# ChristophReich1996/Multi-StyleGAN

Measured on AMD Instinct MI355X. Metric: training images/sec (G+D step, 256^2, seq=3x2ch), higher is better.
Workload: dtype bf16

## Files before the change

### include/msg_hip.h

```cpp
#ifndef MSG_HIP_H
#define MSG_HIP_H

#ifdef __cplusplus
extern "C" {
#endif

enum { MSG_OK = 0, MSG_EINVAL = -1, MSG_EUNSUPPORTED = -2, MSG_ELAUNCH = -3 };
enum { MSG_F32 = 0, MSG_BF16 = 1, MSG_F16 = 2, MSG_F64 = 3, MSG_F32_SPLIT = 4 };

#define MSG_ABI_VERSION 5
int msg_abi_version(void);
const char* msg_build_arch(void);
const char* msg_strerror(int code);

int msg_upfirdn2d(const void* x, const float* fir, void* y, int dtype,
                  int major, int in_h, int in_w, int minor, int kh, int kw,
                  int up_x, int up_y, int down_x, int down_y,
                  int pad_x0, int pad_x1, int pad_y0, int pad_y1, void* stream);

int msg_upfirdn2d_pitched(const void* x, const float* fir, void* y, int dtype,
                          int major, int in_h, int in_w, int minor, int in_pitch, int kh, int kw,
                          int up_x, int up_y, int down_x, int down_y,
                          int pad_x0, int pad_x1, int pad_y0, int pad_y1, void* stream);

// ... 54 lines not shown
                     int per_sample, int k_chunks, int oi_major, float gain,
                     float* ws, long long ws_floats, void* stream);
long long msg_conv2d_wgrad_workspace(int dtype, int B, int IH, int IW, int Cx, int I, int OH, int OW, int ldgy,
                                     int O, int ldgw, int kh, int kw, int stride, int pad, int pixel_shuffle,
                                     int per_sample, int k_chunks);

int msg_demod_coeff(const float* W, const float* s, float* d, int B, int O, int I, int taps,
                    float scale, float eps, void* stream);
int msg_scale_rows_cols(const float* base, const float* rowscale, const float* colscale, void* out,
                        int dtype, int B, int R, int T, int C, int Ck, float gain, void* stream);
int msg_modulate_weights(const float* base, const float* wsq, const float* style, void* out, float* d_out,
                         int dtype, int B, int R, int O, int T, int C, int Ck, float scale, float eps, void* stream);
int msg_modulate_backward(const float* gwk, const float* W, const float* s, const float* d, float* gW,
                          float* gs_part, int B, int O, int I, int taps, int ldg, int o_group,
                          float scale, void* stream);
int msg_scale_rows_cols2(const float* base, const float* row1, const float* col1, const float* row2, const float* col2,
                         void* out, int dtype, int B, int R, int T, int C, int Ck, float gain, void* stream);
int msg_modulate_backward2(const float* gwk, const float* W, const float* s, const float* d, const float* v,
                           float* gW, float* gs_part, int B, int O, int I, int taps, int ldg, int o_group,
                           float scale, void* stream);

int msg_relayout_weight(const float* w, void* fwd, void* dgrad, float* wsq, int dtype,
                        int O, int I, int T, int Ck, int Ok, int flip, int t_major, float gain, void* stream);

int msg_gather_taps(const void* x, void* y, int dtype, int B, int H, int W, int Cx, int C, int kh, int kw,
                    int pad, int Ko, void* stream);
int msg_fold_taps(const void* g, const void* add, void* gx, int dtype, int B, int H, int W, int Ko, int C, int kh, int kw,
                  int pad, int ldx, int ld_add, void* stream);

int msg_scaled_add(const void* a, const void* b, void* y, int dtype, long long n, float beta, float gain, void* stream);
int msg_rgb_skip_merge(const void* conv, int dtype, int ld, const float* bias, const float* skip, const float* fir,
                       float* out, int B, int C, int H, int W, void* stream);
int msg_rgb_skip_merge_backward(const float* g, void* g_conv, int dtype, int ld, float* g_skip, const float* fir,
                                int B, int C, int H, int W, void* stream);
int msg_gamma_merge(const void* a, const void* b, const float* gamma, void* y, int dtype, long long n, float gain, void* stream);
long long msg_gamma_merge_backward_workspace(void);
int msg_gamma_merge_backward(const void* gy, const void* a, const float* gamma, void* ga, void* gb, float* g_gamma, int dtype,
                             long long n, float gain, float* ws, void* stream);
int msg_scaled_add_rows(const void* a, const void* b, void* y, int dtype, long long rows, int cols,
                        long long lda, long long ldb, long long ldy, float beta, float gain, void* stream);

int msg_softmax_rows(const void* x, void* y, int dtype, long long rows, int cols, void* stream);
int msg_softmax_rows_backward(const void* y, const void* gy, void* gx, int dtype, long long rows, int cols,
                              void* stream);
int msg_softmax_rows_backward2(const void* y, const void* gy, const void* v, void* d_y, void* d_gy, int dtype,
                               long long rows, int cols, void* stream);

int msg_nonlocal_attention_supported(int B, int Nq, int Nk, int dk, int dv);
int msg_nonlocal_attention_fwd(const void* q, const void* k, const void* vt, void* o, float* lse, int dtype,
                               int B, int Nq, int Nk, int dk, int dv, void* stream);
int msg_maxpool2x2_fwd(const void* x, void* y, unsigned short* idx, int dtype, int B, int H, int W, int C, long long ldx,
                       void* stream);
int msg_maxpool2x2_bwd(const void* gy, const unsigned short* idx, void* gx, int dtype, int B, int H, int W, int C,
                       void* stream);
int msg_maxpool2x2_gather(const void* v, const unsigned short* idx, void* out, int dtype, int B, int H, int W, int C,
                          long long ldv, void* stream);

int msg_nonlocal_attention_bwd_splits(int B, int Nq, int Nk);
int msg_nonlocal_attention_bwd(const void* q, const void* qt, const void* k, const void* kt, const void* v,
                               const void* dO, const void* dOt, const void* o, const float* lse, float* delta,
                               void* dq, void* dk_out, void* dv_out, float* workspace, int dtype,
                               int B, int Nq, int Nk, int dk, int dv, void* stream);

int msg_affine_warp(const float* x, float* y, const float* angle_deg, float angle_const, const float* scale_xy,
                    const float* select_u, const float* p, int rot_prob, float cx, float cy, int padding,
                    int align_corners, int B, int C, int H, int W, int backward, void* workspace, void* stream);

long long msg_minibatch_stddev_workspace(int C, int H, int W, int groups, int dtype);
int msg_minibatch_stddev(const void* x, void* y, float* stat, float* workspace, int dtype,
                         int B, int C, int H, int W, int ldx, int ldy, int groups, float alpha, void* stream);
int msg_minibatch_stddev_backward(const void* x, const void* gy, const float* gstat, void* gx, int dtype,
                                  int B, int C, int H, int W, int ldx, int ldgy, int ldgx, int groups,
                                  float alpha, void* stream);

int msg_conv2d_fprop_act(const void* x, const void* w, void* y, int dtype,
                         int B, int IH, int IW, int Cx, int Ck, int OH, int OW, int N, int ldy,
                         int kh, int kw, int stride, int pad, long long w_batch_stride,
                         const float* act_bias, const float* noise, const float* noise_weight,
                         int noise_batch, float alpha, float scale, void* stream);
int msg_conv2d_fprop_act_mask(const void* x, const void* w, void* y, int dtype,
                              int B, int IH, int IW, int Cx, int Ck, int OH, int OW, int N, int ldy,
                              int kh, int kw, int stride, int pad, long long w_batch_stride,
                              const float* act_bias, const float* noise, const float* noise_weight,
                              int noise_batch, float alpha, float scale, unsigned char* mask, void* stream);

int msg_conv2d_fprop_residual(const void* x, const void* w, void* y, int dtype,
                              int B, int IH, int IW, int Cx, int Ck, int OH, int OW, int N, int ldy,
                              int kh, int kw, int stride, int pad, long long w_batch_stride,
                              const void* residual, int res_ld, float gain, void* stream);

int msg_conv2d_fprop_act_backward(const void* x, const void* w, void* y, int dtype,
                                  int B, int IH, int IW, int Cx, int Ck, int OH, int OW, int N, int ldy,
                                  int kh, int kw, int stride, int pad, long long w_batch_stride,
                                  const void* residual, int res_ld,
                                  const unsigned char* sign_mask, int mask_tile_m, int mask_tile_n,
                                  const void* sign_map, int sign_ld, float alpha, float scale,
                                  float* grad_bias, const float* noise, int noise_batch, float* grad_noise_weight,
                                  float* ws, long long ws_floats, void* stream);

int msg_act_pointwise_head(const void* x, const float* bias, const float* w, float* y, int dtype,
                           long long npix, int C, float wscale, float alpha, float scale, void* stream);
long long msg_act_pointwise_head_backward_workspace(long long npix, int C);
int msg_act_pointwise_head_backward(const void* x, const float* bias, const float* w, const float* gy, void* gx,
                                    float* grad_bias_and_w, int dtype, long long npix, int C, float wscale,
                                    float alpha, float scale, float* ws, long long ws_floats, void* stream);

int msg_linear_fprop(const float* x, const float* w, const float* bias, float* y, int M, int N, int K,
                     float gain, float bias_gain, void* stream);
int msg_linear_dgrad(const float* gy, const float* w, float* gx, int M, int N, int K, float gain, void* stream);
int msg_linear_wgrad(const float* gy, const float* x, float* gw, float* gb, int M, int N, int K,
                     float gain, float bias_gain, void* stream);

int msg_linear_grouped_fprop(const float* x, const int* slot, const float* const* w, const float* const* bias, float* y,
                             int G, int M, int N, int K, int L, float gain, float bias_gain, void* stream);
int msg_linear_grouped_dgrad(const float* gy, const float* const* w, float* gx, int G, int M, int N, int K, float gain,
                             void* stream);
int msg_linear_grouped_wgrad(const float* gy, const float* x, const int* slot, float* gw, float* gb, int G, int M, int N,
                             int K, int L, float gain, float bias_gain, void* stream);
int msg_linear_grouped_wgrad_ptrs(const float* gy, const float* x, const int* slot, float* const* gw, float* const* gb, int G,
                                  int M, int N, int K, int L, float gain, float bias_gain, void* stream);

enum {
    MSG_PLAN_REG = 0,
    MSG_PLAN_DMA = 1,
    MSG_PLAN_PP = 2,
    MSG_PLAN_ROW3 = 3,
    MSG_PLAN_ROW3N = 4,
    MSG_PLAN_THIN = 5,
    MSG_PLAN_UPCONV = 6,
    MSG_FPLAN_FIELDS = 5
};
int msg_conv2d_fprop_launch_plan(int dtype, int B, int IH, int IW, int Cx, int Ck, int OH, int OW, int N, int ldy,
                                 int kh, int kw, int stride, int pad, int in_up, int pixel_shuffle,
                                 long long w_batch_stride, int has_bias, int epilogue, long long* out, int n_out_fields);
enum {
    MSG_WPLAN_GENERIC = 0,
    MSG_WPLAN_DMA = 1,
    MSG_WPLAN_UNI = 2,
    MSG_WPLAN_ROW3 = 3,
    MSG_WPLAN_ROW3_W32 = 4,
    MSG_WPLAN_FIELDS = 11
};
int msg_conv2d_wgrad_plan(int dtype, int B, int IH, int IW, int Cx, int I, int OH, int OW, int ldgy,
                          int O, int ldgw, int kh, int kw, int stride, int pad, int pixel_shuffle,
                          int per_sample, int k_chunks, long long* out, int n_out_fields);
int msg_conv2d_fprop_plan(int dtype, int B, int IH, int IW, int Cx, int Ck, int OH, int OW, int N,
                          int kh, int kw, long long w_batch_stride);
long long msg_conv2d_fprop_act_backward_workspace(int dtype, int B, int IH, int IW, int Cx, int Ck, int OH, int OW,
                                                  int N, int kh, int kw, long long w_batch_stride, int has_noise);
int msg_conv2d_fprop_upconv_eligible(int B, int IH, int IW, int Cx, int Ck, int OH, int OW, int N, int kh, int kw,
                                     int stride, int pad, int in_up, int pixel_shuffle, long long w_batch_stride);
int msg_conv2d_fprop_thin_eligible(int B, int IH, int IW, int Cx, int Ck, int OH, int OW, int N, int ldy, int kh, int kw,
                                   int stride, int pad, int in_up, int pixel_shuffle, int act_mode);

int msg_flat_adam(float* param, const float* grad, float* exp_avg, float* exp_avg_sq, float* ema, long long n,
                  const float* coef, float lr, float beta1, float beta2, float eps, int step, float ema_decay,
                  void* stream);
int msg_flat_ema(float* ema, const float* param, long long n, float decay, void* stream);

long long msg_tlfm_prepare_workspace(int B, int T);
int msg_tlfm_prepare(const unsigned short* raw, const unsigned char* hflip, void* out, int dtype,
                     int B, int C, int T, int H, int W, int vflip,
                     float lo1, float div1, float lo2, float div2,
                     unsigned int* ws, void* stream);

int msg_tlfm_frame_range(const unsigned short* frames, long long N, int H, int W,
                         unsigned int* range, void* stream);
int msg_tlfm_gather(const unsigned short* frames, const unsigned int* range, long long N,
                    const int* index, const unsigned char* hflip, void* out, int dtype,
                    int B, int C, int T, int H, int W, int vflip,
                    float lo1, float div1, float lo2, float div2, void* stream);

long long msg_tlfm_export_workspace(int B, int T);
int msg_tlfm_export(const void* x, int dtype, const int* bf_range, unsigned short* out,
                    int B, int C, int T, int H, int W, int vflip, int bf_normalise,
                    float low1, float div1, float low2, float div2,
                    float* ws, void* stream);

int msg_sample_sheet(const void* seq, unsigned char* out, int dtype,
                     int B, int C, int T, int H, int W, int tints, void* stream);

enum { MSG_GAN_LOGISTIC = 0, MSG_GAN_WASSERSTEIN = 1, MSG_GAN_HINGE = 2 };
enum { MSG_GAN_AUX_NONE = 0, MSG_GAN_AUX_WEIGHT = 1, MSG_GAN_AUX_LABEL = 2 };
long long msg_gan_loss_workspace(long long n_real, long long n_fake);
int msg_gan_loss(const void* pred_real, const void* pred_fake, const float* aux, float* out, int dtype, int kind,
                 int aux_mode, long long n_real, long long n_fake, long long P, float* ws, long long ws_floats,
                 void* stream);
int msg_gan_loss_backward(const void* pred_real, const void* pred_fake, const float* aux, const float* grad_out,
                          void* grad_real, void* grad_fake, int dtype, int kind, int aux_mode,
                          long long n_real, long long n_fake, long long P, void* stream);

#define MSG_ELASTIC_MAX_SIGMA 32
long long msg_elastic_workspace(int B, int H, int W);
int msg_elastic_deform(const void* in, const float* noise, float* field, void* out, int dtype,
                       int B, int F, int H, int W, int sigma, float alpha, void* ws, void* stream);

#define MSG_JPEG_MAX_WIDTH 16384
long long msg_jpeg_workspace(int N, int H, int W);
int msg_jpeg_scan_capacity(int N, int H, int W, long long* bytes);
int msg_jpeg_encode(const unsigned char* rgb, const unsigned short* qtables, short* coef, unsigned char* scan,
                    long long* offsets, int N, int H, int W, void* ws, void* stream);

enum { MSG_METRIC_NORM_NONE = 0, MSG_METRIC_NORM_SOURCE = 1, MSG_METRIC_NORM_RESIZED = 2 };
#define MSG_METRIC_MAX_SCALE 8
long long msg_metric_input_workspace(int B, int T, int H, int W, int t, int out_h, int out_w, int norm);
int msg_metric_input(const void* images, int in_dtype, int B, int C, int T, int H, int W,
                     int channel, int t, void* out, int out_dtype, int planes,
                     int out_h, int out_w, int norm, void* ws, void* stream);

#ifdef __cplusplus
}
#endif
#endif
```

### multi_stylegan_amd/csrc/conv_dispatch.h

```cpp
#pragma once
#include "msg_common.h"

struct ConvProblem {
    int dtype;
    int split;
    int B, IH, IW, Cx, Ck, OH, OW, N, ldy;
    int kh, kw, stride, pad, in_up, pixel_shuffle;
    long long w_batch_stride;

    bool per_sample() const { return w_batch_stride != 0; }
    int samples() const { return per_sample() ? B : 1; }
    long long mtot() const { return per_sample() ? (long long)OH * OW : (long long)B * OH * OW; }
    int esz() const { return dtype == MSG_BF16 ? 2 : 4; }
    long long x_bstride() const { return (long long)IH * IW * Cx; }
    long long y_bstride() const { return (pixel_shuffle ? 4ll : 1ll) * OH * OW * ldy; }
    long long x_bytes() const { return (long long)(per_sample() ? 1 : B) * IH * IW * Cx * esz(); }
    long long w_bytes() const { return (long long)N * kh * kw * Ck * esz(); }
    bool fits31() const { return x_bytes() < 0x7ffffff0ll && w_bytes() < 0x7ffffff0ll; }
};

enum ConvKernel {
    CONV_THIN_N, CONV_THIN_K,
    CONV_UPCONV,
    CONV_ROW3, CONV_ROW3N,
    CONV_PP,
    CONV_DMA, CONV_REG, CONV_REG_LEAN, CONV_REG_SPLIT
};

struct ConvPlan {
    ConvKernel kernel;
    int tile_m, tile_n;
    bool supported;
};

inline int conv_act_mode(const ActEpilogue* act) { return act ? act->enabled : 0; }

template <typename P>
inline void conv_fill_common(P& p, const ConvProblem& q, const ActEpilogue* act) {
    p.B = q.B; p.IH = q.IH; p.IW = q.IW; p.Cx = q.Cx; p.Ck = q.Ck; p.OH = q.OH; p.OW = q.OW; p.N = q.N; p.ldy = q.ldy;
    p.per_sample = q.per_sample();
    if (act) p.act = *act;
    p.x_bstride = q.x_bstride();
    p.w_bstride = q.w_batch_stride;
    p.y_bstride = q.y_bstride();
    p.Mtot = (int)q.mtot();
}
template <typename P>
inline void conv_fill_taps(P& p, const ConvProblem& q) {
    p.kh = q.kh; p.kw = q.kw; p.stride = q.stride; p.pad = q.pad; p.in_up = q.in_up; p.pixel_shuffle = q.pixel_shuffle;
}

ConvPlan conv_fprop_select(const ConvProblem& q, const ActEpilogue* act, bool has_bias);

bool conv_thin_eligible(const ConvProblem& q, const ActEpilogue* act, ConvPlan* plan);
void conv_thin_launch(const ConvProblem& q, const ConvPlan& plan, const void* x, const void* w, const float* bias, void* y,
                      const ActEpilogue* act, void* stream);
bool conv_upconv_eligible(const ConvProblem& q, const ActEpilogue* act, bool has_bias, ConvPlan* plan);
void conv_upconv_launch(const ConvProblem& q, const ConvPlan& plan, const void* x, const void* w, void* y, void* stream);
bool conv_row3_eligible(const ConvProblem& q, const ActEpilogue* act, bool has_bias, ConvPlan* plan);
void conv_row3_launch(const ConvProblem& q, const ConvPlan& plan, const void* x, const void* w, const float* bias, void* y,
                      const ActEpilogue* act, void* stream);
bool conv_pp_eligible(const ConvProblem& q, ConvPlan* plan);
void conv_pp_launch(const ConvProblem& q, const ConvPlan& plan, const void* x, const void* w, const float* bias, void* y,
                    const ActEpilogue* act, void* stream);

struct WgradProblem {
    int dtype, split;
    int B, IH, IW, Cx, I, OH, OW, ldgy, O, ldgw;
    int kh, kw, stride, pad, pixel_shuffle;
    int per_sample, k_chunks, oi_major;
    float gain;
    int esz() const { return dtype == MSG_BF16 ? 2 : 4; }
    long long gy_bytes() const { return (long long)(pixel_shuffle ? 4 : 1) * OH * OW * ldgy * esz(); }
    long long x_bytes() const { return (long long)IH * IW * Cx * esz(); }
    long long slab() const { return (long long)O * kh * kw * ldgw; }
    long long gw_zstride() const { return oi_major ? (long long)O * I * kh * kw : slab(); }
};

enum WgradKernel {
    WGRAD_GENERIC, WGRAD_DMA, WGRAD_UNI,
    WGRAD_ROW3, WGRAD_ROW3_W32
};

struct WgradPlan {
    WgradKernel kernel;
    int nz, slice_pixels;
    int chunks_per_out, n_out;
    int OWv, OHv;
    int fold, xcd_slices;
    long long blocks, need;
    bool supported;
};

struct WgradSplitModel { int round_wgs, fixed_steps, slab_steps; long long max_chunks, max_wgs; bool by8; };
inline long long conv_wgrad_ksplit(long long steps, long long wgs, const WgradSplitModel& m) {
    long long chunks = 1, best = -1;
    for (long long c = 1; c <= m.max_chunks; c += (m.by8 && c >= 8 ? 8 : 1)) {
        if (m.by8 && c > 1 && c < 8) continue;
        const long long rounds = (wgs * c + m.round_wgs - 1) / m.round_wgs;
        const long long cost = rounds * ((steps + c - 1) / c + m.fixed_steps + (c > 1 ? m.slab_steps : 0));
        if (best < 0 || cost < best) { best = cost; chunks = c; }
        if (wgs * c > m.max_wgs) break;
    }
    return chunks;
}

inline int conv_wgrad_default_chunks(const WgradProblem& q) {
    const long long kp = q.dtype == MSG_BF16 ? 64 : 32, npix = (long long)q.OH * q.OW;
    long long tiles = (long long)((q.O + 127ll) / 128) * ((q.I + 127ll) / 128);
    for (const int n : {q.kh, q.kw, q.B}) tiles = tiles < 1024 ? tiles * n : 1024;
    if (q.per_sample) {
        if (tiles >= 256) return 1;
        return (int)std::max(1ll, std::min(npix / (16 * kp), 1024 / tiles));
    }
    long long chunks = std::max(1ll, std::min((npix + 4 * kp - 1) / (4 * kp), (1024 + tiles - 1) / tiles));
    while (q.B * chunks > 65535) --chunks;
    return (int)chunks;
}

WgradPlan conv_wgrad_select(const WgradProblem& q);
bool conv_wgrad_row3_eligible(const WgradProblem& q, WgradPlan* plan);
void conv_wgrad_row3_launch(const WgradProblem& q, const WgradPlan& plan, const void* gy, const void* x, float* gw, float* ws,
                            void* stream);
```

### multi_stylegan_amd/csrc/conv_fprop.hip

```cpp
#include "conv_dispatch.h"
#include <stdlib.h>

typedef __bf16 bf16v8 __attribute__((ext_vector_type(8)));
typedef const __attribute__((address_space(1))) char* gptr_t;
typedef const __attribute__((address_space(1))) u32x4* gvec_t;
typedef __attribute__((address_space(3))) char* lds_t;

struct ConvParams {
    int B, IH, IW, Cx, Ck, OH, OW, N, ldy;
    int kh, kw, stride, pad, in_up, pixel_shuffle, per_sample;
    long long x_bstride, w_bstride, y_bstride;
    int Mtot, n_chunks, n_iters, m_tiles, n_tiles;
    ActEpilogue act;
};

constexpr int BM = 128, BN = 128, ROWB = 128;
constexpr int STAGE_BYTES = (BM + BN) * ROWB;
__device__ __attribute__((aligned(256))) unsigned int g_zero_page[16384];

__device__ __forceinline__ int swz(int row, int slot) { return row * ROWB + ((slot ^ ((row >> 1) & 7)) << 4); }

template <int SPLIT>
__device__ __forceinline__ void split_park(const u32x4& raw, char* dst) {
    uint2 pl[3];
// ... 235 lines not shown
                }
#pragma unroll
                for (int e = 0; e < 4; ++e)
#pragma unroll
                    for (int i = 0; i < 2; ++i)
#pragma unroll
                        for (int j = 0; j < 2; ++j)
                            acc[i][j] = __builtin_amdgcn_mfma_f32_32x32x2f32(fb[j][e], fa[i][e], acc[i][j], 0, 0, 0);
            }
        }
    };
    if constexpr (ONE_STAGE) {
        load_next();
        for (int it = 0; it < p.n_iters; ++it) {
            if (it) __syncthreads();
            park(0);
            if (it + 1 < p.n_iters) load_next();
            __syncthreads();
            mma_step(smem);
        }
    } else {
        if constexpr (DMA) {
            dma_stage = 0;
            load_next();
        } else {
            load_next();
            park(0);
            if (p.n_iters > 1) load_next();
        }
        for (int it = 0; it < p.n_iters; ++it) {
            if constexpr (DMA) asm volatile("s_waitcnt vmcnt(0)" ::: "memory");
            __syncthreads();
            if constexpr (DMA) {
                if (it + 1 < p.n_iters) { dma_stage = (it + 1) & 1; load_next(); }
            } else {
                if (it + 1 < p.n_iters) park((it + 1) & 1);
                if (it + 2 < p.n_iters) load_next();
            }
            mma_step(smem + (it & 1) * STAGE);
        }
    }
    if constexpr (DMA) asm volatile("s_waitcnt vmcnt(0)" ::: "memory");
    __syncthreads();

    constexpr int PITCH = 64 * sizeof(T);
    constexpr int UNITB = 4 * sizeof(T);
    char* ep = smem + wid * (64 * PITCH);
#pragma unroll
    for (int j = 0; j < 2; ++j)
#pragma unroll
        for (int g = 0; g < 4; ++g) {
            const int unit = 8 * j + 2 * g + lh;
            float bv[4] = {0.f, 0.f, 0.f, 0.f};
            if (bias) {
                const int nb = n0 + wn * 64 + 4 * unit;
#pragma unroll
                for (int e = 0; e < 4; ++e) bv[e] = nb + e < p.N ? bias[nb + e] : 0.f;
            }
#pragma unroll
            for (int i = 0; i < 2; ++i) {
                const int row = i * 32 + lr;
                char* dstl = ep + row * PITCH + ((unit ^ (row & 15)) * UNITB);
                if constexpr (sizeof(T) == 2) {
                    uint2 pk;
                    pk.x = (unsigned)f2bf(acc[i][j][4 * g + 0] + bv[0]) | ((unsigned)f2bf(acc[i][j][4 * g + 1] + bv[1]) << 16);
                    pk.y = (unsigned)f2bf(acc[i][j][4 * g + 2] + bv[2]) | ((unsigned)f2bf(acc[i][j][4 * g + 3] + bv[3]) << 16);
                    *reinterpret_cast<uint2*>(dstl) = pk;
                } else {
                    *reinterpret_cast<f32x4*>(dstl) = f32x4{acc[i][j][4 * g + 0] + bv[0], acc[i][j][4 * g + 1] + bv[1],
                                                            acc[i][j][4 * g + 2] + bv[2], acc[i][j][4 * g + 3] + bv[3]};
                }
            }
        }
    constexpr int LPR = 64 / VEC;
    constexpr int RPP = 64 / LPR;
    constexpr int NPASS = 64 / RPP;
    const int er = lane / LPR, ec = (lane % LPR) * VEC;
    const int n = n0 + wn * 64 + ec;
    int nn = n, q = 0;
    if (p.pixel_shuffle) { const int oc = p.N >> 2; q = n / oc; nn = n - q * oc; }
    const int lim = p.pixel_shuffle ? (p.N >> 2) - nn : p.N - n;
    const bool n_ok = n < p.N;
    int gp[NPASS];
    float a_bias[VEC], a_noise[NPASS];
    {
        const int m_first = min(m0 + wm * 64 + er, p.Mtot - 1);
        int b = p.per_sample ? bz : m_first / ohw;
        const int pix0 = p.per_sample ? m_first : m_first - b * ohw;
        int oh = pix0 / p.OW, ow = pix0 - oh * p.OW;
        const bool want_noise = p.act.enabled == 1 && p.act.noise;
        const float nw = want_noise ? p.act.noise_w[0] : 0.f;
        if (p.act.enabled == 1) {
#pragma unroll
            for (int e = 0; e < VEC; ++e) a_bias[e] = (p.act.bias && n + e < p.N) ? p.act.bias[n + e] : 0.f;
        }
#pragma unroll
        for (int pass = 0; pass < NPASS; ++pass) {
            const bool ok = m0 + wm * 64 + pass * RPP + er < p.Mtot;
            const int pix = oh * p.OW + ow;
            const int g = p.pixel_shuffle ? ((b * 2 * p.OH + 2 * oh + (q >> 1)) * (2 * p.OW) + 2 * ow + (q & 1))
                                          : b * ohw + pix;
            gp[pass] = ok ? g : -1;
            a_noise[pass] = (want_noise && ok) ? nw * p.act.noise[(long long)(p.act.noise_batch == 1 ? 0 : b) * ohw + pix] : 0.f;
            ow += RPP;
            while (ow >= p.OW) { ow -= p.OW; ++oh; }
            if (!p.per_sample) while (oh >= p.OH) { oh -= p.OH; ++b; }
        }
    }
    __syncthreads();
    u32x4 v[NPASS];
#pragma unroll
    for (int pass = 0; pass < NPASS; ++pass) {
        const int row = pass * RPP + er;
        if constexpr (sizeof(T) == 2)
            v[pass] = *reinterpret_cast<const u32x4*>(ep + row * PITCH + (((lane & 7) ^ ((row & 15) >> 1)) << 4));
        else
            v[pass] = *reinterpret_cast<const u32x4*>(ep + row * PITCH + (((lane & 15) ^ (row & 15)) << 4));
    }
    if constexpr (sizeof(T) == 2) {
        if (er & 1) {
#pragma unroll
            for (int pass = 0; pass < NPASS; ++pass) v[pass] = u32x4{v[pass][2], v[pass][3], v[pass][0], v[pass][1]};
        }
    }
    if (p.act.enabled == 1) {
#pragma unroll
        for (int pass = 0; pass < NPASS; ++pass) v[pass] = act_epilogue_apply<T>(v[pass], a_bias, a_noise[pass], p.act.alpha, p.act.scale);
    } else if (p.act.enabled == 2) {
        const T* rbase = reinterpret_cast<const T*>(p.act.residual) + (n_ok ? n : 0);
        u32x4 r[NPASS];
#pragma unroll
        for (int pass = 0; pass < NPASS; ++pass)
            r[pass] = *reinterpret_cast<const u32x4*>(rbase + (long long)max(gp[pass], 0) * p.act.res_ld);
#pragma unroll
        for (int pass = 0; pass < NPASS; ++pass) v[pass] = residual_epilogue_apply<T>(v[pass], r[pass], p.act.res_gain);
    }
    T* ybase = y + (p.pixel_shuffle ? nn : n);
    if (n_ok && lim >= VEC) {
#pragma unroll
        for (int pass = 0; pass < NPASS; ++pass)
            if (gp[pass] >= 0) *reinterpret_cast<u32x4*>(ybase + (long long)gp[pass] * p.ldy) = v[pass];
    } else if (n_ok) {
#pragma unroll
        for (int pass = 0; pass < NPASS; ++pass) {
            if (gp[pass] < 0) continue;
            T tmp[VEC];
            *reinterpret_cast<u32x4*>(tmp) = v[pass];
            T* dst = ybase + (long long)gp[pass] * p.ldy;
            for (int e = 0; e < lim; ++e) dst[e] = tmp[e];
        }
    }
}

static ConvPlan conv_generic_select(const ConvProblem& q) {
    const int n_iters = q.kh * q.kw * (q.Ck / (ROWB / q.esz()));
    static const int variant = msg_tunable("MSG_CONV_VARIANT", 0);
    const bool dma = q.fits31() && (variant == 1 || (variant == 0 && n_iters >= 8));
    static const int lean_max = msg_tunable("MSG_CONV_LEAN", 4);
    ConvPlan plan{CONV_REG, BM, BN, true};
    if (q.split) plan.kernel = CONV_REG_SPLIT;
    else if (dma) plan.kernel = CONV_DMA;
    else if (q.dtype == MSG_BF16 && n_iters <= lean_max) plan.kernel = CONV_REG_LEAN;
    const long long mtot = q.mtot(), blocks = ((mtot + BM - 1) / BM) * ((q.N + BN - 1) / BN);
    plan.supported = mtot < (1ll << 31) && blocks < (1ll << 31) &&
                     (long long)(n_iters + 1) * ROWB + 128 <= 65536;
    return plan;
}

static void conv_generic_launch(const ConvProblem& q, const ConvPlan& plan, const void* x, const void* w, const float* bias, void* y,
                                const ActEpilogue* act, void* stream) {
    ConvParams p{};
    conv_fill_common(p, q, act);
    conv_fill_taps(p, q);
    p.n_chunks = q.Ck / (ROWB / q.esz());
    p.n_iters = q.kh * q.kw * p.n_chunks;
    p.m_tiles = (int)((q.mtot() + BM - 1) / BM);
    p.n_tiles = (q.N + BN - 1) / BN;
    dim3 grid((unsigned)((long long)p.m_tiles * p.n_tiles), 1, q.samples());
#define GENERIC(T, ...) hipLaunchKernelGGL((conv_fprop_kernel<T, __VA_ARGS__>), grid, dim3(256), 0, (hipStream_t)stream, \
                                           (const T*)x, (const T*)w, (T*)y, bias, p)
    const bool bf16 = q.dtype == MSG_BF16;
    if (bf16 && plan.kernel == CONV_REG_LEAN) GENERIC(bf16_t, false, 3);
    else if (bf16 && plan.kernel == CONV_DMA) GENERIC(bf16_t, true);
    else if (bf16) GENERIC(bf16_t, false);
    else if (plan.kernel == CONV_REG_SPLIT) GENERIC(float, false, 0, 3);
    else if (plan.kernel == CONV_DMA) GENERIC(float, true);
    else GENERIC(float, false);
#undef GENERIC
}

ConvPlan conv_fprop_select(const ConvProblem& q, const ActEpilogue* act, bool has_bias) {
    ConvPlan plan;
    if (conv_thin_eligible(q, act, &plan)) return plan;
    if (conv_upconv_eligible(q, act, has_bias, &plan)) return plan;
    if (conv_row3_eligible(q, act, has_bias, &plan)) return plan;
    if (conv_pp_eligible(q, &plan)) return plan;
    return conv_generic_select(q);
}

static ConvProblem conv_problem(int dtype, int B, int IH, int IW, int Cx, int Ck, int OH, int OW, int N, int ldy,
                                int kh, int kw, int stride, int pad, int in_up, int pixel_shuffle, long long w_batch_stride) {
    const int split = dtype == MSG_F32_SPLIT ? 3 : 0;
    return ConvProblem{split ? (int)MSG_F32 : dtype, split, B, IH, IW, Cx, Ck, OH, OW, N, ldy, kh, kw, stride, pad, in_up, pixel_shuffle,
                       w_batch_stride};
}

static ConvPlan fprop_select(const ConvProblem& q, int act_mode, bool has_bias) {
    ActEpilogue act{};
    act.enabled = act_mode;
    return conv_fprop_select(q, &act, has_bias);
}

static int fprop_check(const ConvProblem& q, const void* const* io) {
    if (q.B < 0 || q.IH <= 0 || q.IW <= 0 || q.OH <= 0 || q.OW <= 0 || q.N <= 0 || q.kh <= 0 || q.kw <= 0 || q.stride <= 0 ||
        q.in_up <= 0 || q.Cx <= 0 || q.Ck <= 0 || q.ldy <= 0 || (io && (!io[0] || !io[1] || !io[2])))
        return MSG_EINVAL;
    if (q.dtype != MSG_F32 && q.dtype != MSG_BF16) return MSG_EUNSUPPORTED;
    const int vec = 16 / q.esz(), bke = ROWB / q.esz();
    if (q.Ck % bke || q.Cx % vec || (io && (((uintptr_t)io[0] | (uintptr_t)io[1] | (uintptr_t)io[2]) & 15u))) return MSG_EUNSUPPORTED;
    if (q.ldy % vec || (q.pixel_shuffle && (q.N % 4 || (q.N / 4) % vec))) return MSG_EUNSUPPORTED;
    if (q.in_up > 1 && q.stride != 1) return MSG_EUNSUPPORTED;
    return MSG_OK;
}

static int fprop_plan_for(const ConvProblem& q, int act_mode, bool has_bias, const void* const* io, ConvPlan* plan) {
    if (q.B == 0) return MSG_OK;
    const int rc = fprop_check(q, io);
    if (rc != MSG_OK) return rc;
    *plan = fprop_select(q, act_mode, has_bias);
    return plan->supported ? MSG_OK : MSG_EUNSUPPORTED;
}

static bool is_row3(const ConvPlan& plan) { return plan.kernel == CONV_ROW3 || plan.kernel == CONV_ROW3N; }

static void act_backward_partials(const ConvProblem& q, const ConvPlan& plan, long long* rows, long long* entries) {
    *rows = *entries = 0;
    if (!is_row3(plan) || q.ldy != q.N) return;
    const long long tiles = (q.mtot() / plan.tile_m) * q.samples();
    *rows = tiles * 2;
    *entries = tiles * (q.N / plan.tile_n) * 4;
}

static int plan_code(ConvKernel kernel) {
    switch (kernel) {
        case CONV_THIN_N: case CONV_THIN_K: return MSG_PLAN_THIN;
        case CONV_UPCONV: return MSG_PLAN_UPCONV;
        case CONV_ROW3: return MSG_PLAN_ROW3;
        case CONV_ROW3N: return MSG_PLAN_ROW3N;
        case CONV_PP: return MSG_PLAN_PP;
        case CONV_DMA: return MSG_PLAN_DMA;
        default: return MSG_PLAN_REG;
    }
}

extern "C" int msg_conv2d_fprop_launch_plan(int dtype, int B, int IH, int IW, int Cx, int Ck, int OH, int OW, int N, int ldy,
                                            int kh, int kw, int stride, int pad, int in_up, int pixel_shuffle,
                                            long long w_batch_stride, int has_bias, int epilogue, long long* out, int n_out_fields) {
    if (epilogue < 0 || epilogue > 3 || (epilogue && (has_bias || in_up != 1 || pixel_shuffle))) return MSG_EINVAL;
    const ConvProblem q = conv_problem(dtype, B, IH, IW, Cx, Ck, OH, OW, N, ldy, kh, kw, stride, pad, in_up, pixel_shuffle, w_batch_stride);
    ConvPlan plan;
    const int rc = fprop_plan_for(q, epilogue, has_bias != 0, nullptr, &plan);
    if (rc != MSG_OK) return rc;
    long long fields[MSG_FPLAN_FIELDS] = {};
    if (q.B) {
        fields[0] = plan_code(plan.kernel); fields[1] = plan.tile_m; fields[2] = plan.tile_n;
        if (epilogue == 3) act_backward_partials(q, plan, &fields[3], &fields[4]);
    }
    for (int k = 0; k < MSG_FPLAN_FIELDS && k < n_out_fields; ++k) out[k] = fields[k];
    return MSG_OK;
}

static ConvProblem conv_query_problem(int dtype, int B, int IH, int IW, int Cx, int Ck, int OH, int OW, int N, int kh, int kw,
                                      long long w_batch_stride) {
    return conv_problem(dtype, B, IH, IW, Cx, Ck, OH, OW, N, N <= 8 ? 8 : (N + 7) / 8 * 8, kh, kw, 1, kh / 2, 1, 0, w_batch_stride);
}
extern "C" int msg_conv2d_fprop_plan(int dtype, int B, int IH, int IW, int Cx, int Ck, int OH, int OW, int N,
                                     int kh, int kw, long long w_batch_stride) {
    return plan_code(fprop_select(conv_query_problem(dtype, B, IH, IW, Cx, Ck, OH, OW, N, kh, kw, w_batch_stride), 0, false).kernel);
}
extern "C" long long msg_conv2d_fprop_act_backward_workspace(int dtype, int B, int IH, int IW, int Cx, int Ck, int OH, int OW,
                                                             int N, int kh, int kw, long long w_batch_stride, int has_noise) {
    const ConvProblem q = conv_query_problem(dtype, B, IH, IW, Cx, Ck, OH, OW, N, kh, kw, w_batch_stride);
    long long rows, entries;
    act_backward_partials(q, fprop_select(q, 3, false), &rows, &entries);
    return rows ? rows * N + (has_noise ? entries : 0) : 0;
}
extern "C" int msg_conv2d_fprop_upconv_eligible(int B, int IH, int IW, int Cx, int Ck, int OH, int OW, int N, int kh, int kw,
                                                int stride, int pad, int in_up, int pixel_shuffle, long long w_batch_stride) {
    return fprop_select(conv_problem(MSG_BF16, B, IH, IW, Cx, Ck, OH, OW, N, N / 4, kh, kw, stride, pad, in_up, pixel_shuffle,
                                     w_batch_stride), 0, false).kernel == CONV_UPCONV;
}
extern "C" int msg_conv2d_fprop_thin_eligible(int B, int IH, int IW, int Cx, int Ck, int OH, int OW, int N, int ldy,
                                              int kh, int kw, int stride, int pad, int in_up, int pixel_shuffle,
                                              int act_mode) {
    const ConvKernel kernel = fprop_select(conv_problem(MSG_BF16, B, IH, IW, Cx, Ck, OH, OW, N, ldy, kh, kw, stride, pad, in_up,
                                                        pixel_shuffle, 0), act_mode, false).kernel;
    return kernel == CONV_THIN_N ? 1 : kernel == CONV_THIN_K ? 2 : 0;
}

static int conv2d_fprop_impl(const void* x, const void* w, const float* bias, void* y, const ConvProblem& q,
                             const ActEpilogue& act, void* stream) {
    const void* const io[3] = {x, w, y};
    ConvPlan plan;
    const int rc = fprop_plan_for(q, act.enabled, bias != nullptr, io, &plan);
    if (rc != MSG_OK || q.B == 0) return rc;
    if (act.mask && !is_row3(plan)) return MSG_EUNSUPPORTED;
    switch (plan.kernel) {
        case CONV_THIN_N: case CONV_THIN_K: conv_thin_launch(q, plan, x, w, bias, y, &act, stream); break;
        case CONV_UPCONV: conv_upconv_launch(q, plan, x, w, y, stream); break;
        case CONV_ROW3: case CONV_ROW3N: conv_row3_launch(q, plan, x, w, bias, y, &act, stream); break;
        case CONV_PP: conv_pp_launch(q, plan, x, w, bias, y, &act, stream); break;
        case CONV_DMA: case CONV_REG: case CONV_REG_LEAN: case CONV_REG_SPLIT:
            conv_generic_launch(q, plan, x, w, bias, y, &act, stream); break;
    }
    return MSG_CHECK_LAUNCH();
}

extern "C" int msg_conv2d_fprop(const void* x, const void* w, const float* bias, void* y, int dtype,
                                int B, int IH, int IW, int Cx, int Ck, int OH, int OW, int N, int ldy,
                                int kh, int kw, int stride, int pad, int in_up, int pixel_shuffle,
                                long long w_batch_stride, void* stream) {
    ActEpilogue act{};
    return conv2d_fprop_impl(x, w, bias, y, conv_problem(dtype, B, IH, IW, Cx, Ck, OH, OW, N, ldy, kh, kw, stride, pad, in_up,
                                                         pixel_shuffle, w_batch_stride), act, stream);
}

extern "C" int msg_conv2d_fprop_act_mask(const void* x, const void* w, void* y, int dtype,
                                         int B, int IH, int IW, int Cx, int Ck, int OH, int OW, int N, int ldy,
                                         int kh, int kw, int stride, int pad, long long w_batch_stride,
                                         const float* act_bias, const float* noise, const float* noise_weight,
                                         int noise_batch, float alpha, float scale, unsigned char* mask, void* stream) {
    if (noise && (!noise_weight || (noise_batch != 1 && noise_batch != B))) return MSG_EINVAL;
    ActEpilogue act{act_bias, noise, noise_weight, noise_batch, 1, alpha, scale, nullptr, 0, 0.f, mask};
    return conv2d_fprop_impl(x, w, nullptr, y, conv_problem(dtype, B, IH, IW, Cx, Ck, OH, OW, N, ldy, kh, kw, stride, pad, 1, 0,
                                                            w_batch_stride), act, stream);
}

extern "C" int msg_conv2d_fprop_act(const void* x, const void* w, void* y, int dtype,
                                    int B, int IH, int IW, int Cx, int Ck, int OH, int OW, int N, int ldy,
                                    int kh, int kw, int stride, int pad, long long w_batch_stride,
                                    const float* act_bias, const float* noise, const float* noise_weight,
                                    int noise_batch, float alpha, float scale, void* stream) {
    return msg_conv2d_fprop_act_mask(x, w, y, dtype, B, IH, IW, Cx, Ck, OH, OW, N, ldy, kh, kw, stride, pad, w_batch_stride,
                                     act_bias, noise, noise_weight, noise_batch, alpha, scale, nullptr, stream);
}

extern "C" int msg_conv2d_fprop_residual(const void* x, const void* w, void* y, int dtype,
                                         int B, int IH, int IW, int Cx, int Ck, int OH, int OW, int N, int ldy,
                                         int kh, int kw, int stride, int pad, long long w_batch_stride,
                                         const void* residual, int res_ld, float gain, void* stream) {
    if (!residual || res_ld < N || (((uintptr_t)residual) & 15u) || res_ld % (dtype == MSG_BF16 ? 8 : 4)) return MSG_EINVAL;
    ActEpilogue act{};
    act.enabled = 2; act.residual = residual; act.res_ld = res_ld; act.res_gain = gain;
    return conv2d_fprop_impl(x, w, nullptr, y, conv_problem(dtype, B, IH, IW, Cx, Ck, OH, OW, N, ldy, kh, kw, stride, pad, 1, 0,
                                                            w_batch_stride), act, stream);
}

extern "C" int msg_conv2d_fprop_act_backward(const void* x, const void* w, void* y, int dtype,
                                             int B, int IH, int IW, int Cx, int Ck, int OH, int OW, int N, int ldy,
                                             int kh, int kw, int stride, int pad, long long w_batch_stride,
                                             const void* residual, int res_ld,
                                             const unsigned char* sign_mask, int mask_tile_m, int mask_tile_n,
                                             const void* sign_map, int sign_ld, float alpha, float scale,
                                             float* grad_bias, const float* noise, int noise_batch, float* grad_noise_weight,
                                             float* ws, long long ws_floats, void* stream) {
    if (B == 0) return MSG_OK;
    if (!sign_mask == !sign_map) return MSG_EINVAL;
    const ConvProblem q = conv_problem(dtype, B, IH, IW, Cx, Ck, OH, OW, N, ldy, kh, kw, stride, pad, 1, 0, w_batch_stride);
    const void* const io[3] = {x, w, y};
    ConvPlan plan;
    const int rc = fprop_plan_for(q, 3, false, io, &plan);
    if (rc != MSG_OK) return rc;
    long long rows, entries;
    act_backward_partials(q, plan, &rows, &entries);
    if (!rows) return MSG_EUNSUPPORTED;
    if (sign_mask && (mask_tile_m <= 0 || mask_tile_n <= 0 || mask_tile_n % 128 || N % mask_tile_n || (((uintptr_t)sign_mask) & 15u) ||
                      (mask_tile_m != 1 && mask_tile_m % 64) || ((long long)B * OH * OW) % mask_tile_m))
        return MSG_EINVAL;
    if (sign_map && (sign_ld < N || sign_ld % 8 || (((uintptr_t)sign_map) & 15u))) return MSG_EINVAL;
    if (residual && (res_ld < N || res_ld % 8 || (((uintptr_t)residual) & 15u))) return MSG_EINVAL;
    const bool has_noise = noise && grad_noise_weight;
    if (has_noise && noise_batch != 1 && noise_batch != B) return MSG_EINVAL;
    const long long need_b = grad_bias ? rows * N : 0, need_n = has_noise ? entries : 0;
    if (need_b + need_n > 0 && (!ws || ws_floats < need_b + need_n)) return MSG_EINVAL;
    ActEpilogue act{};
    act.enabled = 3; act.alpha = alpha; act.scale = scale;
    act.residual = residual; act.res_ld = res_ld; act.res_gain = 1.f;
    act.mask = const_cast<unsigned char*>(sign_mask); act.mask_tile_m = mask_tile_m; act.mask_tile_n = mask_tile_n;
    act.sign_src = sign_map; act.sign_ld = sign_ld;
    act.noise = has_noise ? noise : nullptr; act.noise_batch = noise_batch;
    act.part_b = grad_bias ? ws : nullptr;
    act.part_n = has_noise ? ws + need_b : nullptr;
    conv_row3_launch(q, plan, x, w, nullptr, y, &act, stream);
    if (MSG_CHECK_LAUNCH() != MSG_OK) return MSG_ELAUNCH;
    return msg_bias_act_reduce_launch(act.part_b, grad_bias, N, rows, act.part_n, grad_noise_weight, entries, stream);
}
```

Baseline: 155.6.

## Add persistent streaming 1x1 conv kernel with LDS-resident weight panel

Adds a specialized bf16 1x1 convolution forward kernel for large pixel counts. Each workgroup keeps a swizzled weight panel in LDS and persistent waves stream 32-pixel blocks with double-buffered register loads, MFMA 32x32x16, and a coalesced LDS-transposed epilogue with optional bias and residual add. It is selected ahead of the lean register kernel when the generic path would not use DMA, aiming to cut repeated weight loads and improve streaming bandwidth. The cost is new code paths and occupancy sized from a runtime query.

Result: no change. 156.7, median of 6 (+0.7%).

```diff
diff --git a/include/msg_hip.h b/include/msg_hip.h
--- a/include/msg_hip.h
+++ b/include/msg_hip.h
@@ -230,6 +230,9 @@
                                      int stride, int pad, int in_up, int pixel_shuffle, long long w_batch_stride);
 int msg_conv2d_fprop_thin_eligible(int B, int IH, int IW, int Cx, int Ck, int OH, int OW, int N, int ldy, int kh, int kw,
                                    int stride, int pad, int in_up, int pixel_shuffle, int act_mode);
+int msg_conv2d_fprop_stream1x1_eligible(int dtype, int B, int IH, int IW, int Cx, int Ck, int OH, int OW, int N, int ldy,
+                                        int kh, int kw, int stride, int pad, int in_up, int pixel_shuffle,
+                                        long long w_batch_stride, int has_bias, int epilogue);
 
 int msg_flat_adam(float* param, const float* grad, float* exp_avg, float* exp_avg_sq, float* ema, long long n,
                   const float* coef, float lr, float beta1, float beta2, float eps, int step, float ema_decay,
diff --git a/multi_stylegan_amd/csrc/conv_dispatch.h b/multi_stylegan_amd/csrc/conv_dispatch.h
--- a/multi_stylegan_amd/csrc/conv_dispatch.h
+++ b/multi_stylegan_amd/csrc/conv_dispatch.h
@@ -24,7 +24,8 @@
     CONV_UPCONV,
     CONV_ROW3, CONV_ROW3N,
     CONV_PP,
-    CONV_DMA, CONV_REG, CONV_REG_LEAN, CONV_REG_SPLIT
+    CONV_DMA, CONV_REG, CONV_REG_LEAN, CONV_REG_SPLIT,
+    CONV_STREAM1X1
 };
 
 struct ConvPlan {
@@ -63,6 +64,9 @@
 bool conv_pp_eligible(const ConvProblem& q, ConvPlan* plan);
 void conv_pp_launch(const ConvProblem& q, const ConvPlan& plan, const void* x, const void* w, const float* bias, void* y,
                     const ActEpilogue* act, void* stream);
+bool conv_stream1x1_eligible(const ConvProblem& q, const ActEpilogue* act, ConvPlan* plan);
+void conv_stream1x1_launch(const ConvProblem& q, const ConvPlan& plan, const void* x, const void* w, const float* bias, void* y,
+                           const ActEpilogue* act, void* stream);
 
 struct WgradProblem {
     int dtype, split;
diff --git a/multi_stylegan_amd/csrc/conv_fprop.hip b/multi_stylegan_amd/csrc/conv_fprop.hip
--- a/multi_stylegan_amd/csrc/conv_fprop.hip
+++ b/multi_stylegan_amd/csrc/conv_fprop.hip
@@ -411,7 +411,7 @@
     }
 }
 
-static ConvPlan conv_generic_select(const ConvProblem& q) {
+static ConvPlan conv_generic_select(const ConvProblem& q, const ActEpilogue* act) {
     const int n_iters = q.kh * q.kw * (q.Ck / (ROWB / q.esz()));
     static const int variant = msg_tunable("MSG_CONV_VARIANT", 0);
     const bool dma = q.fits31() && (variant == 1 || (variant == 0 && n_iters >= 8));
@@ -419,6 +419,7 @@
     ConvPlan plan{CONV_REG, BM, BN, true};
     if (q.split) plan.kernel = CONV_REG_SPLIT;
     else if (dma) plan.kernel = CONV_DMA;
+    else if (conv_stream1x1_eligible(q, act, &plan)) {}
     else if (q.dtype == MSG_BF16 && n_iters <= lean_max) plan.kernel = CONV_REG_LEAN;
     const long long mtot = q.mtot(), blocks = ((mtot + BM - 1) / BM) * ((q.N + BN - 1) / BN);
     plan.supported = mtot < (1ll << 31) && blocks < (1ll << 31) &&
@@ -454,7 +455,7 @@
     if (conv_upconv_eligible(q, act, has_bias, &plan)) return plan;
     if (conv_row3_eligible(q, act, has_bias, &plan)) return plan;
     if (conv_pp_eligible(q, &plan)) return plan;
-    return conv_generic_select(q);
+    return conv_generic_select(q, act);
 }
 
 static ConvProblem conv_problem(int dtype, int B, int IH, int IW, int Cx, int Ck, int OH, int OW, int N, int ldy,
@@ -555,6 +556,15 @@
     const ConvKernel kernel = fprop_select(conv_problem(MSG_BF16, B, IH, IW, Cx, Ck, OH, OW, N, ldy, kh, kw, stride, pad, in_up,
                                                         pixel_shuffle, 0), act_mode, false).kernel;
     return kernel == CONV_THIN_N ? 1 : kernel == CONV_THIN_K ? 2 : 0;
+}
+
+extern "C" int msg_conv2d_fprop_stream1x1_eligible(int dtype, int B, int IH, int IW, int Cx, int Ck, int OH, int OW, int N, int ldy,
+                                                   int kh, int kw, int stride, int pad, int in_up, int pixel_shuffle,
+                                                   long long w_batch_stride, int has_bias, int epilogue) {
+    if (epilogue < 0 || epilogue > 3 || (epilogue && (has_bias || in_up != 1 || pixel_shuffle))) return 0;
+    const ConvProblem q = conv_problem(dtype, B, IH, IW, Cx, Ck, OH, OW, N, ldy, kh, kw, stride, pad, in_up, pixel_shuffle, w_batch_stride);
+    ConvPlan plan;
+    return fprop_plan_for(q, epilogue, has_bias != 0, nullptr, &plan) == MSG_OK && q.B && plan.kernel == CONV_STREAM1X1;
 }
 
 static int conv2d_fprop_impl(const void* x, const void* w, const float* bias, void* y, const ConvProblem& q,
@@ -571,6 +581,7 @@
         case CONV_PP: conv_pp_launch(q, plan, x, w, bias, y, &act, stream); break;
         case CONV_DMA: case CONV_REG: case CONV_REG_LEAN: case CONV_REG_SPLIT:
             conv_generic_launch(q, plan, x, w, bias, y, &act, stream); break;
+        case CONV_STREAM1X1: conv_stream1x1_launch(q, plan, x, w, bias, y, &act, stream); break;
     }
     return MSG_CHECK_LAUNCH();
 }
diff --git a/multi_stylegan_amd/csrc/conv_stream1x1.hip b/multi_stylegan_amd/csrc/conv_stream1x1.hip
--- /dev/null
+++ b/multi_stylegan_amd/csrc/conv_stream1x1.hip
@@ -0,0 +1,193 @@
+#include "conv_dispatch.h"
+
+typedef __bf16 bf16v8 __attribute__((ext_vector_type(8)));
+typedef const __attribute__((address_space(1))) char* gptr_t;
+typedef const __attribute__((address_space(1))) u32x4* gvec_t;
+
+struct Stream1x1Params {
+    int M, n_blocks;
+    int Cx, N, ldy;
+    const float* bias;
+    const void* residual;
+    int res_ld;
+    float res_gain;
+};
+
+constexpr int S1_PIX = 32, S1_WAVES = 4;
+constexpr int S1_PATCH = S1_PIX * 64 * 2;
+constexpr long long S1_MIN_PIXELS = 1ll << 18;
+constexpr int S1_WG_PER_CU = 2, S1_MAX_WG_PER_CU = 4;
+
+__device__ __forceinline__ int s1_swz(int row, int slot) { return row * 128 + ((slot ^ ((row >> 1) & 7)) << 4); }
+
+template <int KT, int NPB, bool RES>
+__global__ __launch_bounds__(64 * S1_WAVES, S1_WG_PER_CU) void conv_stream1x1_kernel(const bf16_t* __restrict__ x,
+                                                                                   const bf16_t* __restrict__ w,
+                                                                                   bf16_t* __restrict__ y, Stream1x1Params p) {
+    constexpr int CK = 16 * KT, NP = 32 * NPB, KC = KT / 4;
+    constexpr int PANEL = NP * CK * 2;
+    static_assert(KT % 4 == 0 && NPB % 2 == 0 && PANEL <= 65536, "whole 128-byte chunks, 64-channel epilogue slices, 64 KiB");
+    __shared__ __attribute__((aligned(16))) char smem[PANEL + S1_WAVES * S1_PATCH];
+    const int tid = threadIdx.x, lane = tid & 63, wid = tid >> 6;
+    const int wid_u = __builtin_amdgcn_readfirstlane(wid);
+    const int lr = lane & 31, lh = lane >> 5;
+    const int n0 = blockIdx.y * NP;
+
+    {
+        const gptr_t wb = (gptr_t)(w + (long long)n0 * CK);
+#pragma unroll 4
+        for (int i = tid; i < NP * KC * 8; i += 64 * S1_WAVES) {
+            const int slot = i & 7, row = (i >> 3) % NP, c = i / (8 * NP);
+            *reinterpret_cast<u32x4*>(smem + c * (NP * 128) + s1_swz(row, slot)) = *(gvec_t)(wb + ((long long)row * CK + c * 64 + slot * 8) * 2);
+        }
+        __syncthreads();
+    }
+    char* patch = smem + PANEL + wid * S1_PATCH;
+    const int gw = blockIdx.x * S1_WAVES + wid_u, n_waves = gridDim.x * S1_WAVES;
+
+    auto load = [&](bf16v8 (&fa)[KT], int blk) __attribute__((always_inline)) {
+        const int m = min(blk * S1_PIX + lr, p.M - 1);
+        const gptr_t src = (gptr_t)x + ((long long)m * p.Cx + 8 * lh) * 2;
+#pragma unroll
+        for (int t = 0; t < KT; ++t) fa[t] = __builtin_bit_cast(bf16v8, *(gvec_t)(src + 32 * t));
+    };
+
+    auto compute = [&](const bf16v8 (&fa)[KT], int blk) __attribute__((always_inline)) {
+        f32x16 acc[NPB];
+#pragma unroll
+        for (int j = 0; j < NPB; ++j)
+#pragma unroll
+            for (int e = 0; e < 16; ++e) acc[j][e] = 0.f;
+#pragma unroll
+        for (int t = 0; t < KT; ++t)
+#pragma unroll
+            for (int j = 0; j < NPB; ++j) {
+                const bf16v8 fb = *reinterpret_cast<const bf16v8*>(smem + (t >> 2) * (NP * 128) + s1_swz(32 * j + lr, 2 * (t & 3) + lh));
+                acc[j] = __builtin_amdgcn_mfma_f32_32x32x16_bf16(fb, fa[t], acc[j], 0, 0, 0);
+            }
+
+        const int er = lane >> 3, ec = lane & 7;
+        const int m0 = blk * S1_PIX;
+        u32x4 r[4];
+        auto load_res = [&](int jp) __attribute__((always_inline)) {
+            const bf16_t* rbase = reinterpret_cast<const bf16_t*>(p.residual) + n0 + 64 * jp + ec * 8;
+#pragma unroll
+            for (int pass = 0; pass < 4; ++pass)
+                r[pass] = *(gvec_t)(gptr_t)(rbase + (long long)min(m0 + pass * 8 + er, p.M - 1) * p.res_ld);
+        };
+        if constexpr (RES) load_res(0);
+#pragma unroll
+        for (int jp = 0; jp < NPB / 2; ++jp) {
+            const int nc = n0 + 64 * jp + ec * 8;
+#pragma unroll
+            for (int jj = 0; jj < 2; ++jj)
+#pragma unroll
+                for (int g = 0; g < 4; ++g) {
+                    const int j = 2 * jp + jj, unit = 8 * jj + 2 * g + lh;
+                    float bv[4] = {0.f, 0.f, 0.f, 0.f};
+                    if (p.bias) {
+                        const int nb = n0 + 64 * jp + 4 * unit;
+#pragma unroll
+                        for (int e = 0; e < 4; ++e) bv[e] = p.bias[nb + e];
+                    }
+                    uint2 pk;
+                    pk.x = (unsigned)f2bf(acc[j][4 * g + 0] + bv[0]) | ((unsigned)f2bf(acc[j][4 * g + 1] + bv[1]) << 16);
+                    pk.y = (unsigned)f2bf(acc[j][4 * g + 2] + bv[2]) | ((unsigned)f2bf(acc[j][4 * g + 3] + bv[3]) << 16);
+                    *reinterpret_cast<uint2*>(patch + lr * 128 + ((unit ^ (lr & 15)) << 3)) = pk;
+                }
+            asm volatile("s_waitcnt lgkmcnt(0)" ::: "memory");
+            u32x4 v[4];
+#pragma unroll
+            for (int pass = 0; pass < 4; ++pass) {
+                const int row = pass * 8 + er;
+                v[pass] = *reinterpret_cast<const u32x4*>(patch + row * 128 + ((ec ^ ((row & 15) >> 1)) << 4));
+                if (row & 1) v[pass] = u32x4{v[pass][2], v[pass][3], v[pass][0], v[pass][1]};
+            }
+            asm volatile("s_waitcnt lgkmcnt(0)" ::: "memory");
+            if constexpr (RES) {
+#pragma unroll
+                for (int pass = 0; pass < 4; ++pass) v[pass] = residual_epilogue_apply<bf16_t>(v[pass], r[pass], p.res_gain);
+                if (jp + 1 < NPB / 2) load_res(jp + 1);
+            }
+#pragma unroll
+            for (int pass = 0; pass < 4; ++pass)
+                *reinterpret_cast<u32x4*>(y + (long long)min(m0 + pass * 8 + er, p.M - 1) * p.ldy + nc) = v[pass];
+        }
+    };
+
+    bf16v8 fa0[KT], fa1[KT];
+    const int last = p.n_blocks - 1;
+    int blk = gw;
+    if (blk >= p.n_blocks) return;
+    load(fa0, blk);
+    load(fa1, min(blk + n_waves, last));
+    compute(fa0, blk);
+    blk += n_waves;
+    while (blk < p.n_blocks) {
+        load(fa0, min(blk + n_waves, last));
+        compute(fa1, blk);
+        blk += n_waves;
+        if (blk >= p.n_blocks) break;
+        load(fa1, min(blk + n_waves, last));
+        compute(fa0, blk);
+        blk += n_waves;
+    }
+}
+
+static int s1_panel_blocks(int Ck, int N) {
+    const int cap = Ck <= 128 ? 8 : 4;
+    for (const int npb : {8, 6, 4, 2})
+        if (npb <= cap && N % (32 * npb) == 0) return npb;
+    return 0;
+}
+
+bool conv_stream1x1_eligible(const ConvProblem& q, const ActEpilogue* act, ConvPlan* plan) {
+    static const int enabled = msg_tunable("MSG_CONV_STREAM1X1", 1);
+    const int mode = conv_act_mode(act);
+    if (!enabled || q.dtype != MSG_BF16 || q.split || q.per_sample()) return false;
+    if (q.kh != 1 || q.kw != 1 || q.stride != 1 || q.pad != 0 || q.in_up != 1 || q.pixel_shuffle) return false;
+    if (q.IH != q.OH || q.IW != q.OW) return false;
+    if (q.Ck != 64 && q.Ck != 128 && q.Ck != 192 && q.Ck != 256) return false;
+    if (q.N % 64 || q.Cx < q.Ck || q.ldy < q.N) return false;
+    if (mode != 0 && mode != 2) return false;
+    if (q.mtot() < S1_MIN_PIXELS || q.mtot() >= (1ll << 31) - S1_PIX) return false;
+    plan->kernel = CONV_STREAM1X1;
+    return true;
+}
+
+void conv_stream1x1_launch(const ConvProblem& q, const ConvPlan&, const void* x, const void* w, const float* bias, void* y,
+                           const ActEpilogue* act, void* stream) {
+    Stream1x1Params p{};
+    p.M = (int)q.mtot();
+    p.n_blocks = (p.M + S1_PIX - 1) / S1_PIX;
+    p.Cx = q.Cx; p.N = q.N; p.ldy = q.ldy;
+    p.bias = bias;
+    const bool res = conv_act_mode(act) == 2;
+    if (res) { p.residual = act->residual; p.res_ld = act->res_ld; p.res_gain = act->res_gain; }
+    const int npb = s1_panel_blocks(q.Ck, q.N), panels = q.N / (32 * npb);
+    static const int cus = [] {
+        int dev = 0, n = 0;
+        return hipGetDevice(&dev) == hipSuccess && hipDeviceGetAttribute(&n, hipDeviceAttributeMultiprocessorCount, dev) == hipSuccess && n > 0 ? n : 256;
+    }();
+    const int blocks4 = (p.n_blocks + S1_WAVES - 1) / S1_WAVES;
+#define S1_LAUNCH(KT_, NPB_, RES_) { \
+        static const int per_cu = [] { \
+            int n = 0; \
+            if (hipOccupancyMaxActiveBlocksPerMultiprocessor(&n, conv_stream1x1_kernel<KT_, NPB_, RES_>, 64 * S1_WAVES, 0) == hipSuccess && n > 0) \
+                return std::min(n, S1_MAX_WG_PER_CU); \
+            (void)hipGetLastError();                     \
+            return S1_WG_PER_CU; \
+        }(); \
+        const dim3 grid(std::max(1, std::min(blocks4, cus * per_cu / panels)), panels); \
+        hipLaunchKernelGGL((conv_stream1x1_kernel<KT_, NPB_, RES_>), grid, dim3(64 * S1_WAVES), 0, (hipStream_t)stream, \
+                           (const bf16_t*)x, (const bf16_t*)w, (bf16_t*)y, p); \
+        return; \
+    }
+#define S1(KT_, NPB_) \
+    if (q.Ck == 16 * KT_ && npb == NPB_) { \
+        if (res) S1_LAUNCH(KT_, NPB_, true) else S1_LAUNCH(KT_, NPB_, false) \
+    }
+    S1(4, 2) S1(4, 4) S1(4, 6) S1(4, 8) S1(8, 2) S1(8, 4) S1(8, 6) S1(8, 8) S1(12, 2) S1(12, 4) S1(16, 2) S1(16, 4)
+#undef S1
+#undef S1_LAUNCH
+}
```
